# dkogan/mrgingham

Measured on AMD Instinct MI355X. Metric: frames/sec, 4096x3072 10x10 board, corner-candidate path (ChESS + level decimation + connected components), frames resident in HBM, higher is better.
Workload: dtype u8->int16 (ChESS), int64/f64 (centroids)

## Files before the change

### mrgingham_amd/csrc/chess_hot.h

```cpp
#pragma once
#include "common.h"
#include "hotlist.h"

namespace mrg {

constexpr int V1_HOTBUF = 768;
constexpr int V1_HOTSEG = V1_HOTBUF / 4;

struct HotSink {
    uint32_t* seg;
    int ys, strip_x;
    int count;
};

__device__ __forceinline__ void expand_records(const HotSink& hs, int nrec, int base, const CompTables& t, int frame) {
    const int lane = threadIdx.x & 63;
    uint32_t* hot = t.hot_xy + (long long)frame * t.cap;
    for (int i0 = 0; i0 < nrec; i0 += 64) {
        const int i = i0 + lane;
        const uint32_t r = i < nrec ? hs.seg[i] : 0u;
        const uint32_t mask = r & 0xffu;
        const int c = __popc(mask);
        int incl = c;
#pragma unroll
        for (int d = 1; d < 64; d <<= 1) {
            const int v = __shfl_up(incl, d);
            if (lane >= d) incl += v;
        }
        const int chunk = __shfl(incl, 63);
        if (c) {
            int k = base + incl - c;
            const int y = hs.ys + (int)(r >> 13), x0 = hs.strip_x + 8 * (int)((r >> 8) & 31u);
            t.gidx[(long long)frame * t.gidx_pitch + (long long)y * t.gw + (x0 >> 3)] = make_uint2((uint32_t)k, mask);
            const uint32_t xy0 = ((uint32_t)y << 16) | (uint32_t)x0;
            uint32_t b = mask;
            while (b) {
                const int j = __ffs(b) - 1;
                b &= b - 1;
                if (k < t.cap) hot[k] = xy0 + (uint32_t)j;
                ++k;
            }
        }
        base += chunk;
    }
}

__device__ __forceinline__ int count_record_pixels(const HotSink& hs, int nrec) {
    const int lane = threadIdx.x & 63;
    int mine = 0;
    for (int i = lane; i < nrec; i += 64) mine += __popc(hs.seg[i] & 0xffu);
#pragma unroll
    for (int d = 32; d >= 1; d >>= 1) mine += __shfl_xor(mine, d);
    return mine;
}

__device__ __forceinline__ void collect_hot(uint32_t bits, int y, int x0, HotSink& hs, const CompTables& t, int frame) {
    const unsigned long long m = __ballot(bits != 0);
    const int rank = (int)__builtin_amdgcn_mbcnt_hi((uint32_t)(m >> 32), __builtin_amdgcn_mbcnt_lo((uint32_t)m, 0));
    const int k = hs.count + rank;
    hs.count += __popcll(m);
    if (bits == 0) return;
    if (k < V1_HOTSEG) {
        hs.seg[k] = bits | ((uint32_t)((x0 - hs.strip_x) >> 3) << 8) | ((uint32_t)(y - hs.ys) << 13);
    } else {
        write_group_direct(t, frame, atomicAdd(t.hot_cnt + frame, __popc(bits)), bits, ((uint32_t)y << 16) | (uint32_t)x0);
    }
}

__device__ __forceinline__ void flush_hot(const HotSink& hs, int* hotcnt, int wave, const CompTables& t, int frame) {
    const int nrec = min(hs.count, V1_HOTSEG);
    const int px = count_record_pixels(hs, nrec);
    __syncthreads();
    if ((threadIdx.x & 63) == 0) hotcnt[wave] = px;
    __syncthreads();
    const int total = hotcnt[0] + hotcnt[1] + hotcnt[2] + hotcnt[3];
    if (total == 0) return;
    if (threadIdx.x == 0) hotcnt[4] = atomicAdd(t.hot_cnt + frame, total);
    __syncthreads();
    int base = hotcnt[4];
    for (int w = 0; w < wave; ++w) base += hotcnt[w];
    expand_records(hs, nrec, base, t, frame);
}

}
```

Measured before the change: 69910.

## Flush hot-pixel segment per wave on overflow and use DPP wave scan

Result: no change. 69390 (-0.7%).

```diff
diff --git a/mrgingham_amd/csrc/chess_hot.h b/mrgingham_amd/csrc/chess_hot.h
--- a/mrgingham_amd/csrc/chess_hot.h
+++ b/mrgingham_amd/csrc/chess_hot.h
@@ -13,21 +13,25 @@
     int count;
 };
 
-__device__ __forceinline__ void expand_records(const HotSink& hs, int nrec, int base, const CompTables& t, int frame) {
-    const int lane = threadIdx.x & 63;
+__device__ __forceinline__ int wave_inclusive_scan(int x) {
+    x += __builtin_amdgcn_update_dpp(0, x, 0x111, 0xf, 0xf, false);
+    x += __builtin_amdgcn_update_dpp(0, x, 0x112, 0xf, 0xf, false);
+    x += __builtin_amdgcn_update_dpp(0, x, 0x114, 0xf, 0xf, false);
+    x += __builtin_amdgcn_update_dpp(0, x, 0x118, 0xf, 0xf, false);
+    x += __builtin_amdgcn_update_dpp(0, x, 0x142, 0xa, 0xf, false);
+    x += __builtin_amdgcn_update_dpp(0, x, 0x143, 0xc, 0xf, false);
+    return x;
+}
+
+__device__ __forceinline__ void expand_records(const HotSink& hs, int nrec, int base, const CompTables& t, int frame, int lane) {
     uint32_t* hot = t.hot_xy + (long long)frame * t.cap;
     for (int i0 = 0; i0 < nrec; i0 += 64) {
         const int i = i0 + lane;
         const uint32_t r = i < nrec ? hs.seg[i] : 0u;
         const uint32_t mask = r & 0xffu;
         const int c = __popc(mask);
-        int incl = c;
-#pragma unroll
-        for (int d = 1; d < 64; d <<= 1) {
-            const int v = __shfl_up(incl, d);
-            if (lane >= d) incl += v;
-        }
-        const int chunk = __shfl(incl, 63);
+        const int incl = wave_inclusive_scan(c);
+        const int chunk = __builtin_amdgcn_readlane(incl, 63);
         if (c) {
             int k = base + incl - c;
             const int y = hs.ys + (int)(r >> 13), x0 = hs.strip_x + 8 * (int)((r >> 8) & 31u);
@@ -45,8 +49,7 @@
     }
 }
 
-__device__ __forceinline__ int count_record_pixels(const HotSink& hs, int nrec) {
-    const int lane = threadIdx.x & 63;
+__device__ __forceinline__ int count_record_pixels(const HotSink& hs, int nrec, int lane) {
     int mine = 0;
     for (int i = lane; i < nrec; i += 64) mine += __popc(hs.seg[i] & 0xffu);
 #pragma unroll
@@ -54,24 +57,34 @@
     return mine;
 }
 
+__device__ __forceinline__ void flush_wave(HotSink& hs, const CompTables& t, int frame) {
+    int lane = threadIdx.x & 63;
+    asm volatile("" : "+v"(lane), "+v"(frame));
+    const int px = count_record_pixels(hs, hs.count, lane);
+    int base = 0;
+    if (lane == 0) base = atomicAdd(t.hot_cnt + frame, px);
+    base = __builtin_amdgcn_readfirstlane(base);
+    asm volatile("" : "+v"(base));
+    expand_records(hs, hs.count, base, t, frame, lane);
+    hs.count = 0;
+}
+
 __device__ __forceinline__ void collect_hot(uint32_t bits, int y, int x0, HotSink& hs, const CompTables& t, int frame) {
     const unsigned long long m = __ballot(bits != 0);
     const int rank = (int)__builtin_amdgcn_mbcnt_hi((uint32_t)(m >> 32), __builtin_amdgcn_mbcnt_lo((uint32_t)m, 0));
+    const int n = __popcll(m);
+    if (__builtin_expect(hs.count + n > V1_HOTSEG, 0)) flush_wave(hs, t, frame);
     const int k = hs.count + rank;
-    hs.count += __popcll(m);
-    if (bits == 0) return;
-    if (k < V1_HOTSEG) {
-        hs.seg[k] = bits | ((uint32_t)((x0 - hs.strip_x) >> 3) << 8) | ((uint32_t)(y - hs.ys) << 13);
-    } else {
-        write_group_direct(t, frame, atomicAdd(t.hot_cnt + frame, __popc(bits)), bits, ((uint32_t)y << 16) | (uint32_t)x0);
-    }
+    hs.count += n;
+    if (bits != 0) hs.seg[k] = bits | ((uint32_t)((x0 - hs.strip_x) >> 3) << 8) | ((uint32_t)(y - hs.ys) << 13);
 }
 
 __device__ __forceinline__ void flush_hot(const HotSink& hs, int* hotcnt, int wave, const CompTables& t, int frame) {
-    const int nrec = min(hs.count, V1_HOTSEG);
-    const int px = count_record_pixels(hs, nrec);
+    const int nrec = hs.count;
+    const int lane = threadIdx.x & 63;
+    const int px = count_record_pixels(hs, nrec, lane);
     __syncthreads();
-    if ((threadIdx.x & 63) == 0) hotcnt[wave] = px;
+    if (lane == 0) hotcnt[wave] = px;
     __syncthreads();
     const int total = hotcnt[0] + hotcnt[1] + hotcnt[2] + hotcnt[3];
     if (total == 0) return;
@@ -79,7 +92,7 @@
     __syncthreads();
     int base = hotcnt[4];
     for (int w = 0; w < wave; ++w) base += hotcnt[w];
-    expand_records(hs, nrec, base, t, frame);
+    expand_records(hs, nrec, base, t, frame, lane);
 }
 
 }
```
